# masa-ue/SVDD

Measured on AMD Instinct MI355X. Metric: decoded sequences/sec (whole node), L=200 M=10 128-step SVDD-MC, higher is better.
Workload: dtype f32; 1 GPU; DNA enhancer SVDD-MC, batch=256/GPU, L=200, M=10, 128 steps (BASELINE.json configs[1]); dilated-CNN backbone 3.3M params + ConvGRU value net; global_batch=256, rng=philox

## Files before the change

### include/svdd_hip.h

```cpp
#ifndef SVDD_HIP_H
#define SVDD_HIP_H

#include <stdint.h>

#ifdef __cplusplus
extern "C" {
#endif

#define SVDD_VOCAB 5
#define SVDD_MASK 4
#define SVDD_MAX_M 1024

enum {
  SVDD_OK = 0,
  SVDD_E_ARG = -1,
  SVDD_E_LAUNCH = -2,
  SVDD_E_NODEVICE = -3
};

enum {
  SVDD_LAYOUT_BLV = 0,
  SVDD_LAYOUT_BVL = 1
};

// ... 134 lines not shown
int svdd_conv_tower_windows_f32(const float* onehot, const float* tiles, const float* bias, const int32_t* win,
                                const float* parent_out, float* out, int n, int L, int M, int nlayers,
                                int residual_mask, const int32_t* live_idx, const int32_t* count, void* stream);

int svdd_candidate_windows_tight(const uint8_t* cand, const uint8_t* x, int B, int L, int M, int margin, int32_t* win,
                                 int32_t* flags, void* on_stream);

int svdd_candidate_parts(const uint8_t* cand, const uint8_t* x, int B, int L, int M, int reach, int gap, int32_t* parts,
                         int32_t* nparts, int32_t* flags, int32_t* key, void* on_stream);
int svdd_conv_tower_parts_f32(const float* onehot, const float* tiles, const float* bias, const int32_t* parts,
                              const float* parent_out, float* out, int n, int L, int M, int nlayers, int residual_mask,
                              int reach, const int32_t* live_idx, const int32_t* count, void* on_stream);

int svdd_backbone_cnn_f32(const uint8_t* x, const float* table0, const float* tiles, const float* vec,
                          const float* w2, float* out, int n, int L, int nlayers, const int* dilations,
                          const int32_t* count, const int32_t* row_idx, int out_scatter, void* stream);
int svdd_backbone_cnn_save_f32(const uint8_t* x, const float* table0, const float* tiles, const float* vec, const float* w2,
                               float* out, int n, int L, int nlayers, const int* dilations, float* xhat, float* rstd,
                               unsigned long long* mask, void* stream);
int svdd_backbone_cnn_grad_f32(const float* dlogits, const float* tiles_bwd, const float* gamma, const float* w2,
                               const float* table0, const float* xhat, const float* rstd, const unsigned long long* mask,
                               float* dx, int n, int L, int nlayers, const int* dilations, void* stream);
int svdd_backbone_incr_f32(const uint8_t* x, const float* table0, const float* tiles, const float* vec, const float* w2,
                           float* out, int n, int L, int nlayers, const int* dilations, int lead, float* planes,
                           uint8_t* x_prev, int32_t* items, unsigned long long* stat, int first, int max_item, void* on_stream);
int svdd_backbone_incr2_f32(const uint8_t* x, const float* table0, const float* tiles, const float* vec, const float* w2,
                            float* out, int n, int L, int nlayers, const int* dilations, int lead, float* planes,
                            uint8_t* x_prev, int32_t* items, unsigned long long* stat, int first, int max_item,
                            int32_t* order, int32_t* order_count, void* on_stream);
int svdd_backbone_incr3_f32(const uint8_t* x, const float* table0, const float* tiles, const float* vec, const float* w2,
                            float* out, int n, int L, int nlayers, const int* dilations, int lead, float* planes,
                            uint8_t* x_prev, int32_t* items, unsigned long long* stat, int first, int max_item,
                            int32_t* order, int32_t* order_count, int depth, void* on_stream);
int svdd_backbone_incr_set_residency(int wg_per_cu);
int svdd_backbone_set_workspace(void* ws, long long bytes);
int svdd_backbone_split_status(int* err);

enum { SVDD_PREC_F32 = 0, SVDD_PREC_F16X3 = 1, SVDD_PREC_BF16X3 = 2, SVDD_PREC_F16 = 3, SVDD_PREC_BF16 = 4 };

int svdd_backbone_cnn_lp(const uint8_t* x, const float* table0, const void* tiles, const float* vec,
                         const float* lscale, const float* w2, float* out, int n, int L, int nlayers,
                         const int* dilations, int prec, const int32_t* count, const int32_t* row_idx, int out_scatter,
                         void* stream);

int svdd_conv_tower_lp(const uint8_t* tok, const void* tiles, const float* bias, const float* inv, void* out,
                       int n, int L, int nlayers, int residual_mask, const int32_t* count, int prec, void* stream);
int svdd_conv_tower_windows_lp(const uint8_t* cand, const void* tiles, const float* bias, const float* inv,
                               const int32_t* win, const void* parent_out, void* out, int n, int L, int M,
                               int nlayers, int residual_mask, const int32_t* live_idx, const int32_t* count,
                               int prec, void* stream);

int svdd_gru_bidir_lp(const float* x, const void* x16, const void* wpack, const float* bpack, const float* inv,
                      float* out, int n, int L, const int32_t* count, int prec, void* stream);

int svdd_value_tail_lp(const float* h_fwd, const float* h_bwd, const void* w1pack, const float* b1,
                       const float* w_eff, const float* b_eff, float inv, float* out, int n, int L, int n_tasks,
                       const int32_t* count, int prec, void* stream);

enum { SVDD_OPT_FORCE_EXACT = 0,
       SVDD_OPT_MSPLIT = 1 ,
       SVDD_OPT_SELECT_ONE_ROW = 2 ,
       SVDD_OPT_BACKBONE_LP_VERSION = 3 ,
       SVDD_OPT_TRUNK_GEMM_VERSION = 4 ,
       SVDD_OPT_CAND_ROW_STRIDE = 5 ,
       SVDD_OPT_TRUNK_PLANES_F32 = 6 ,
       SVDD_OPT_SELECT_BATCHES = 8 ,
// ... 60 lines not shown
```

### svdd_amd/_lib.py

```python
import ctypes
import os
import subprocess

_HERE = os.path.dirname(os.path.abspath(__file__))
CSRC = os.path.join(_HERE, "csrc")
SO_PATH = os.environ.get("SVDD_HIP_LIB") or os.path.join(CSRC, "libsvdd_hip.so")
ABI_VERSION = 17

OK, E_ARG, E_LAUNCH, E_NODEVICE = 0, -1, -2, -3
LAYOUT_BLV, LAYOUT_BVL = 0, 1
RNG_REPLAY, RNG_PHILOX = 0, 1
SELECT_ARGMAX, SELECT_MULTINOMIAL = 0, 1
TARGET_MEAN, TARGET_LOGMEANEXP = 0, 1
EVOLVE_GLOBAL, EVOLVE_ROW = 0, 1
ATTR_GRADIENT, ATTR_TIMES_INPUT = 0, 1
PRECISIONS = {"f32": 0, "f16x3": 1, "bf16x3": 2, "f16": 3, "bf16": 4}
MAX_M = 1024

OPT_FORCE_EXACT, OPT_MSPLIT, OPT_SELECT_ONE_ROW, OPT_BACKBONE_LP_VERSION, OPT_TRUNK_GEMM_VERSION = 0, 1, 2, 3, 4
OPT_CAND_ROW_STRIDE, OPT_TRUNK_PLANES_F32, OPT_BACKBONE_SPLIT, OPT_SELECT_BATCHES = 5, 6, 7, 8


class SvddRng(ctypes.Structure):
    _fields_ = [("kind", ctypes.c_int32), ("step", ctypes.c_uint32), ("uniforms", ctypes.c_void_p),
# ... 69 lines not shown
    "svdd_bb_layer_fwd_f32": (vp, vp, vp, vp, vp, vp, f32, vp, vp, vp, i64, i32, i32, STREAM),
    "svdd_bb_layer_bwd_f32": (vp, vp, vp, vp, f32, vp, vp, vp, vp, i64, i32, i32, STREAM),
    "svdd_mt19937_uniform_f32": (vp, vp, i64, STREAM),
    "svdd_backbone_set_workspace": (vp, i64),
    "svdd_backbone_split_status": (pi32,),
    "svdd_backbone_cnn_save_f32": (vp, vp, vp, vp, vp, vp, i32, i32, i32, pi32, vp, vp, vp, STREAM),
    "svdd_backbone_cnn_grad_f32": (vp, vp, vp, vp, vp, vp, vp, vp, vp, i32, i32, i32, pi32, STREAM),
    "svdd_dps_probs": (vp, vp, i32, i32, vp, STREAM),
    "svdd_dps_probs_bwd": (vp, vp, vp, i32, i32, vp, vp, STREAM),
    "svdd_dps_guided_q": (vp, vp, vp, vp, f32, f32, f32, i32, i32, vp, STREAM),
    "svdd_reward_stem_f32": (vp, vp, vp, vp, i32, i32, i32, STREAM),
    "svdd_reward_stem_bwd_f32": (vp, vp, vp, i32, i32, i32, STREAM),
    "svdd_conv1d_cl_gated_f32": (vp, vp, vp, i32, i32, i32, i32, i32, i32, vp, vp, STREAM),
    "svdd_reward_tail_grad_f32": (vp, vp, vp, vp, vp, vp, vp, f32, i32, i32, vp, vp, STREAM),
    "svdd_sum_gate_f32": (vp, vp, vp, vp, i64, STREAM),
    "svdd_gru_bidir_train2_f32": (vp, vp, vp, vp, vp, vp, i32, i32, STREAM),
    "svdd_gru_bidir_bwd2_f32": (vp, vp, vp, vp, vp, vp, vp, i32, i32, STREAM),
    "svdd_classifier_propose": (vp, i32, vp, vp, f32, f32, f32, i32, i32, RNG, vp, vp, vp, STREAM),
    "svdd_elbo_mask": (vp, i32, i32, i32, f64, RNG, vp, vp, vp, vp, vp, vp, STREAM),
    "svdd_elbo_nll": (vp, i32, vp, vp, vp, i32, i32, i32, vp, vp, vp, vp, STREAM),
    "svdd_refine_remask": (vp, vp, vp, vp, vp, f32, i32, i32, RNG, vp, vp, vp, vp, vp, vp, vp),
    "svdd_value_target": (vp, vp, i32, i32, i32, i32, f32, vp, vp, vp, vp),
    "svdd_ism_mutants": (vp, vp, vp, i32, i32, i32, vp, vp, vp, vp),
    "svdd_ism_fold": (vp, vp, vp, vp, vp, vp, i32, i32, i32, i32, i32, vp, vp, vp, vp, vp),
    "svdd_evolve_apply": (vp, vp, vp, i32, i32, i32, vp, vp, vp, vp, vp, vp, vp, vp, vp, vp, vp, vp),
    "svdd_attr_path": (vp, vp, i32, vp, i32, i32, i32, i32, i32, i32, vp, vp, vp),
    "svdd_attr_fold": (vp, f32, vp, vp, vp, i32, i32, i32, i32, i32, i32, i32, vp, vp, vp, vp),
    "svdd_candidate_windows_tight": (vp, vp, i32, i32, i32, i32, vp, vp, vp),
    "svdd_kmer_counts": (vp, i32, i32, i32, vp, vp, vp),
    "svdd_pack_tokens": (vp, i32, i32, vp, vp, vp),
    "svdd_hamming_nn": (vp, vp, i32, i32, i32, i32, i32, i32, vp, vp, vp),
    "svdd_candidate_parts": (vp, vp, i32, i32, i32, i32, i32, vp, vp, vp, vp, vp),
    "svdd_conv_tower_parts_f32": (vp, vp, vp, vp, vp, vp, i32, i32, i32, i32, i32, i32, vp, vp, vp),
}
EXPORTS = tuple(SIGNATURES)


def build(force=False):
    import glob
    srcs = sorted(glob.glob(os.path.join(CSRC, "*.hip")) + glob.glob(os.path.join(CSRC, "*.h")) + [os.path.join(CSRC, "Makefile")])
    srcs.append(os.path.join(os.path.dirname(_HERE), "include", "svdd_hip.h"))
    if os.environ.get("SVDD_HIP_LIB"):
        return SO_PATH
    stale = not os.path.exists(SO_PATH) or os.path.getmtime(SO_PATH) < max(os.path.getmtime(f) for f in srcs)
    if force or stale:
        subprocess.check_call(["make", "-C", CSRC, "-B", "-j", str(min(8, os.cpu_count() or 1))])
    return SO_PATH


_lib = None


def lib():
    global _lib
    if _lib is not None:
        return _lib
    import torch
    if not os.path.exists(SO_PATH):
        raise SvddError(f"{SO_PATH} is missing: build it with `python -c 'import __graft_entry__ as g; g.build()'` "
                        "or `make -C svdd_amd/csrc`. There is no CPU fallback for the SVDD hot path.")
    L = ctypes.CDLL(SO_PATH)
    for name in EXPORTS:
        if not hasattr(L, name):
            raise SvddError(f"libsvdd_hip.so does not export {name}")
    if L.svdd_abi_version() != ABI_VERSION:
        raise SvddError(f"libsvdd_hip.so ABI {L.svdd_abi_version()} != binding ABI {ABI_VERSION}; rebuild")
# ... 102 lines not shown
```

### svdd_amd/csrc/svdd_nets.hip

```cpp
#include "svdd_host.h"

namespace {

typedef float f32x4 __attribute__((ext_vector_type(4)));

__device__ __forceinline__ float wave_sum(float v) {
#pragma unroll
  for (int off = 32; off > 0; off >>= 1) v += __shfl_xor(v, off, 64);
  return v;
}


constexpr int H = 64;
constexpr int HPAD = H + 4;

__device__ __forceinline__ float sigmoid_fast(float a) {
  return __builtin_amdgcn_rcpf(1.0f + __builtin_amdgcn_exp2f(-1.44269504088896f * a));
}
__device__ __forceinline__ float tanh_fast(float a) {
  return 1.0f - 2.0f * __builtin_amdgcn_rcpf(1.0f + __builtin_amdgcn_exp2f(2.88539008177793f * a));
}

template <bool BOTH>
__global__ __launch_bounds__(BOTH ? 512 : 256) void gru_bidir_kernel(const float* __restrict__ x, const float* __restrict__ wpack,
// ... 1994 lines not shown
    int run = 0;
    for (int c = 0; c < 4; ++c) { base[c] = run; run += wtot[0][c] + wtot[1][c] + wtot[2][c] + wtot[3][c]; }
    order_count[blockIdx.x] = run;
  }
  __syncthreads();
  for (int r0 = 0; r0 < n; r0 += 256) {
    const int r = r0 + tid;
    int item[SLOTS], pos[4];
    for (int c = 0; c < 4; ++c) cnt[c] = 0;
    for (int s = 0; s < SLOTS; ++s) {
      item[s] = r < n ? it[r * SLOTS + s] : 0;
      for (int c = 0; c < 4; ++c) cnt[c] += (item[s] >> 8) == 4 - c;
    }
    for (int c = 0; c < 4; ++c) {
      int v = cnt[c];
#pragma unroll
      for (int off = 1; off < 64; off <<= 1) { const int u = __shfl_up(v, off, 64); if (lane >= off) v += u; }
      pos[c] = v - cnt[c];
      if (lane == 63) wtot[w][c] = v;
    }
    __syncthreads();
    for (int c = 0; c < 4; ++c) {
      int at = base[c] + pos[c];
      for (int q = 0; q < w; ++q) at += wtot[q][c];
      for (int s = 0; s < SLOTS; ++s)
        if ((item[s] >> 8) == 4 - c) ord[at++] = r << 16 | item[s];
    }
    __syncthreads();
    if (tid < 4) base[tid] += wtot[0][tid] + wtot[1][tid] + wtot[2][tid] + wtot[3][tid];
    __syncthreads();
  }
}

template <int NC, bool ORD = false, int DIL = 1>
__global__ __launch_bounds__(256, NC == 4 ? 2 : NC == 1 ? 4 : 3) void backbone_seg_kernel(BackboneSegArgs a) {
  static_assert(DIL == 1 || DIL == 4, "one halo tile per side holds taps of dilation <= 4");
  constexpr int NS = NC + 2, ROWS = 16 * NS;
  extern __shared__ __attribute__((aligned(16))) float smem[];
  float* img = smem;
  float* psum = img + ROWS * BB_AP;
  float* rstat = psum + 4 * ROWS;
  int* toks = reinterpret_cast<int*>(rstat + ROWS);

  int item, seq;
  if (ORD) {
    if ((int)blockIdx.x >= a.order_count[a.layer - 1]) return;
    const unsigned ent = (unsigned)__builtin_amdgcn_readfirstlane(a.order[(size_t)(a.layer - 1) * a.order_stride + blockIdx.x]);
    item = (int)(ent & 0xFFFFu);
    seq = (int)(ent >> 16);
  } else {
    item = __builtin_amdgcn_readfirstlane(a.items[(size_t)(a.layer - 1) * a.n * SEG_SLOTS + blockIdx.x]);
    seq = blockIdx.x / SEG_SLOTS;
  }
  const int nown = min(item >> 8, NC);
  if (nown == 0) return;
  const int t0 = item & 255;
  const int tid = threadIdx.x, lane = tid & 63;
  const int cg = __builtin_amdgcn_readfirstlane(tid >> 6);
  const int j = lane & 15, g = lane >> 4;
  const int col0 = 32 * cg + j;
  const int L = a.L;
  const int r0 = 16 * (t0 - 1);
  const size_t pl_stride = (size_t)a.n * TW_ROWS * BB_C;
  float* pl0 = a.planes + (size_t)seq * TW_ROWS * BB_C;
  const int cl = a.layer - 1;
#define SEG_LIVE(S) ((S) <= nown + 1)
// ... 176 lines not shown
        SG_MM(0, UC)                                                                                         \
      } else {                                                                                               \
        SG_MM(0, ua)                                                                                         \
        SG_ALOAD(0, ua, dbytes2)                                                                             \
        SG_MM(1, ub)                                                                                         \
        SG_ALOAD(1, ub, dbytes2)                                                                             \
      }                                                                                                      \
      ++it; }
  float4 ua[2], ub[2];
  SG_ALOAD(0, ua, SG_DBYTES(0))
  if constexpr (NC > 1) SG_ALOAD(1, ub, SG_DBYTES(0))
  for (int it = 0; it < 36;) {
    SG_ENTRY(bA, bB, ua, ub)
    SG_ENTRY(bB, bA, ub, ua)
  }
#undef SG_ENTRY
#undef SG_MM
#undef SG_ALOAD
#undef SG_DBYTES

  float* dst = pl0 + (size_t)cl * pl_stride;
#pragma unroll
  for (int c = 0; c < NC; ++c) {
    if (c >= nown) continue;
#pragma unroll
    for (int ct = 0; ct < 2; ++ct)
#pragma unroll
      for (int e = 0; e < 4; ++e) {
        const int row = r0 + 16 * (c + 1) + 4 * g + e;
        if (row < L) dst[row * BB_C + col0 + 16 * ct] = fmaxf(cacc[c][ct][e], 0.0f) + f[c + 1][ct][e];
      }
  }
#undef SEG_LIVE
}

struct BackboneGradArgs {
  const float* dlogits;
  const float* tiles;
  const float* gamma;
  const float* w2;
  const float* table0;
  float* dx;
  int n, L, nl;
  int dil[BB_MAXL];
};

__global__ __launch_bounds__(512, 2) void backbone_grad_kernel(BackboneGradArgs a, BackboneSave sv) {
  extern __shared__ __attribute__((aligned(16))) float smem[];
  float* img = smem + BB_AP;
  float* Bs = smem + (TW_ROWS + 2) * BB_AP;
  float* psum = Bs + 9 * 5 * BB_C;
  float* rstat = psum + 8 * TW_ROWS;
  int* sdil = reinterpret_cast<int*>(rstat + 2 * TW_ROWS);
  int* sched = sdil + BB_MAXL + 1;

  const int tid = threadIdx.x, lane = tid & 63;
  const int w = __builtin_amdgcn_readfirstlane(tid >> 6);
  const int cg = w & 3, rh = w >> 2;
  const int j = lane & 15, g = lane >> 4;
  const int col0 = 32 * cg + j;
  const int L = a.L, nl = a.nl;
  const int tile_rows = L;
  const int64_t row0 = (int64_t)blockIdx.x * L;
  const int it_end = (nl + 1) * 36;
  constexpr int NR = 7;

// ... 1001 lines not shown
  if (first) {
    if (hipMemcpyAsync(x_prev, x, (size_t)n * L, hipMemcpyDeviceToDevice, (hipStream_t)stream) != hipSuccess) return SVDD_E_LAUNCH;
    return svdd_launch_timed(span.all(), backbone_kernel<true, false, 1>, dim3((unsigned)n), dim3(512), lds, stream, a, BackboneSave{});
  }
  const int slots = max_item == 1 ? TW_RT : SEG_SLOTS;
  if (svdd_launch_timed(span.first(), max_item == 1 ? backbone_worklist_kernel<TW_RT> : backbone_worklist_kernel<SEG_SLOTS>,
                        dim3((unsigned)((n + 3) / 4)), dim3(256), 0, stream, x, x_prev, n, L, depth, max_item, items, stat,
                        backbone_reach(dilations, depth, lead)) != SVDD_OK)
    return SVDD_E_LAUNCH;
  if (svdd_launch(max_item == 1 ? backbone_order_kernel<TW_RT> : backbone_order_kernel<SEG_SLOTS>, dim3((unsigned)depth), dim3(256), 0, stream,
                  items, n, order, order_count) != SVDD_OK)
    return SVDD_E_LAUNCH;
  BackboneSegArgs sa{x, table0, tiles, vec, planes, items, n, L, 0, order, order_count, n * slots};
  const int rows = 16 * (max_item + 2);
  size_t slds = sizeof(float) * ((size_t)rows * BB_AP + 5 * (size_t)rows + rows + 8);
  if (g_incr_residency > 0) {
    const size_t pad = (CU_LDS_BYTES / (size_t)(g_incr_residency + 1) / 1024 + 1) * 1024;
    if (pad > slds) slds = pad;
  }
  const dim3 sgrid((unsigned)(n * slots));
  void (*seg1)(BackboneSegArgs) = max_item == 4 ? backbone_seg_kernel<4, true> : max_item == 2 ? backbone_seg_kernel<2, true>
                                                                                                 : backbone_seg_kernel<1, true>;
  void (*seg4)(BackboneSegArgs) = max_item == 4 ? backbone_seg_kernel<4, true, 4> : max_item == 2 ? backbone_seg_kernel<2, true, 4>
                                                                                                    : backbone_seg_kernel<1, true, 4>;
  svdd_raise_lds_limit(seg1, slds);
  if (depth > lead) svdd_raise_lds_limit(seg4, slds);
  for (int k = 1; k <= depth; ++k) {
    sa.layer = k;
    if (svdd_launch(k <= lead ? seg1 : seg4, sgrid, dim3(256), slds, stream, sa) != SVDD_OK) return SVDD_E_LAUNCH;
  }
  return svdd_launch_timed(span.last(), backbone_kernel<true, false, 2>, dim3((unsigned)n), dim3(512), lds, stream, a, BackboneSave{});
}

typedef decltype(&value_tail_kernel<1>) ValueTailKernel;

extern "C" int svdd_value_tail_f32(const float* h_fwd, const float* h_bwd, const float* w1pack, const float* b1,
                                   const float* w_eff, const float* b_eff, float* out, int n, int L, int n_tasks,
                                   const int32_t* count, void* stream) {
  if (!h_fwd || !h_bwd || !w1pack || !b1 || !w_eff || !b_eff || !out || n <= 0 || L <= 0 || n_tasks < 1 || n_tasks > 4)
    return SVDD_E_ARG;
  ValueTailKernel kern;
  switch (n_tasks) {
    case 1: kern = value_tail_kernel<1>; break;
    case 2: kern = value_tail_kernel<2>; break;
    case 3: kern = value_tail_kernel<3>; break;
    default: kern = value_tail_kernel<4>; break;
  }
  SvddSpan span(SVDD_SLOT_VALUE_TAIL);
  return svdd_launch_timed(span.all(), kern, dim3((unsigned)((n + 3) / 4)), dim3(256), 0, stream, h_fwd, h_bwd, w1pack, b1, w_eff, b_eff, out,
                           n, L, count);
}

extern "C" int svdd_candidate_windows(const uint8_t* cand, const uint8_t* x, int B, int L, int M, int margin, int32_t* win,
                                      int32_t* flags, void* stream) {
  if (!cand || !x || !win || B <= 0 || L <= 0 || M <= 0 || margin < 0) return SVDD_E_ARG;
  const int n = B * M;
  return svdd_launch(candidate_windows_kernel<false>, dim3((unsigned)((n + 3) / 4)), dim3(256), 0, stream, cand, x, n, L, M, margin, win, flags);
}

extern "C" int svdd_candidate_windows_tight(const uint8_t* cand, const uint8_t* x, int B, int L, int M, int margin, int32_t* win,
                                            int32_t* flags, void* on_stream) {
  if (!cand || !x || !win || B <= 0 || L <= 0 || M <= 0 || margin < 0 || margin > (1 << 20) ||
      (long long)B * M > 0x7fffffffLL)
    return SVDD_E_ARG;
  const int n = B * M;
  return svdd_launch(candidate_windows_kernel<true>, dim3((unsigned)((n + 3) / 4)), dim3(256), 0, on_stream, cand, x, n, L, M, margin, win, flags);
// ... 36 lines not shown
```

### svdd_amd/diffusion.py

```python
import contextlib
import functools
import math
import os
import warnings
import weakref
from dataclasses import dataclass
from typing import Optional

import numpy as np
import torch
import torch.nn.functional as F
from torch import nn

from . import noise_schedule, ops
from .backbone import CNNModel


@dataclass
class Loss:
    loss: torch.Tensor
    nlls: torch.Tensor
    token_mask: torch.Tensor


# ... 99 lines not shown
            self.backbone = CNNModel(config.model, alphabet_size=self.vocab_size, num_cls=3)
        elif config.backbone == "dit":
            from .dit import DIT
            self.backbone = DIT(config.model, vocab_size=self.vocab_size)
        else:
            raise ValueError(f"Unknown backbone: {config.backbone}")
        if self.parameterization != "subs":
            raise ValueError("only the `subs` parameterization is on the reference's decode path "
                             "(configs_gosai/config_gosai.yaml:13)")
        self.T = config.T
        self.subs_masking = config.subs_masking
        self.noise = noise_schedule.get_noise(config)
        self.time_conditioning = config.time_conditioning
        self.neg_infinity = -1000000.0
        self.sampling_eps = config.training.sampling_eps
        self.rng_mode = "replay"
        self.value_batching = "batched"
        self.select_mode = "argmax"
        self.philox_seed = 0
        self.row_offset = 0
        self._shard = None
        self.fuse_nets = True
        self.precision = "f32"
        self.skip_unchanged = True
        self.late_steps_from = "auto"
        self.dedup_prior = True
        self.dps_fused = True
        self.dps_one_launch = True
        self._dps_hard_onehot, self._dps_raw_logits, self._dps_logp = False, None, None
        self.dps_single_forward = False
        self.logits_cache = "auto"
        self.incremental_backbone = "auto"
        self.incremental_depth = os.environ.get("SVDD_INCR_DEPTH") or "auto"
        self.skip_stats = None
        self.skip_generic = False
        self.trace = None
        self.state_trace = None
        self._sched_cache = {}
        self._fused = WeightCache()
        self._scope_depth, self._scope_id = 0, 0
        self.fuse_trunk_f32 = True
        self.replay_rng = "device"
        self._replay_stream = None
        self._replay_checked = None
        self._classifier_fused_last = None
        self.elbo_trace = None
        self._from_state = False
        self.cdq_draws = 10
        self._step_base = 0

    @property
    def device(self):
        return next(self.parameters()).device

    def _require_gpu(self):
        if self.device.type != "cuda":
            raise ops.SvddError("the SVDD sampler runs on the GPU only (move the model with .cuda()); "
                                "there is no CPU fallback for the hot path")

    def _schedule(self, num_steps, eps, t_start=1.0):
        key = (num_steps, eps, float(t_start))
        if key not in self._sched_cache:
            tab, timesteps, dt = noise_schedule.move_chance_table(self.noise, num_steps, eps, float(t_start))
            self._sched_cache[key] = (tab.numpy().copy(), timesteps, dt)
        return self._sched_cache[key]

# ... 1137 lines not shown
        mode, rng = self._select_args(step)
        x_next, _, _, _ = ops.select_compact(sc, ws.slot, ws.parent_score, cand, mode=mode, rng=rng, sel_score=ws.sel_score,
                                             changed=ws.changed, idx=ws.idx)
        ws.parent_score, ws.sel_score = ws.sel_score, ws.parent_score
        if ws.parent_out is not None and ws.seq is not None:
            ops.advance_rows(ws.seq, ws.slot, ws.idx, ws.parent_out, ws.M)
        if self.skip_stats is not None:
            ws.n_live += ws.count
            ws.n_changed += ws.changed.sum()
        return x_next

    def _dense_scores(self, sc, ws, B, M):
        live = ws.slot >= 0
        return torch.where(live, sc[ws.slot.clamp(min=0).long()], ws.parent_score.repeat_interleave(M)).view(B, M)

    def _finish_stats(self, ws, B, M, S, kind):
        if self.skip_stats is not None:
            self.skip_stats.update(kind=kind, steps=S, candidates=B * M * S, live_candidates=int(ws.n_live),
                                   row_steps=B * S, changed_row_steps=int(ws.n_changed),
                                   tower_window_rows=None if ws.n_win_rows is None else int(round(float(ws.n_win_rows))),
                                   tower_tile_layers=None if ws.n_tile_layers is None else int(ws.n_tile_layers))

    def _use_logits_cache(self, L):
        return self.logits_cache == "on" or (self.logits_cache == "auto" and 208 // L >= 2)

    def _incremental_stem(self, B, L):
        if self.incremental_backbone not in ("auto", "on", "off"):
            raise ValueError(f"incremental_backbone = {self.incremental_backbone!r}: expected 'auto', 'on' or 'off'")
        if self.incremental_backbone == "off" or _capturing():
            return None, None
        fb = self._fused_backbone_or_none(L)
        if fb is None or not fb.incremental_ok(B, L, any_batch=self.incremental_backbone == "on"):
            return None, None
        return fb, fb.incremental_stem(B, L, self._incremental_depth(fb))

    def _incremental_depth(self, fb):
        from .fused import INCR_DEPTH_AUTO, leading_dilation1, following_dilation4
        lead = leading_dilation1(fb.ol_dil)
        most = lead + following_dilation4(fb.ol_dil)
        if self.incremental_depth == "auto":
            return min(max(INCR_DEPTH_AUTO, lead), most)
        try:
            depth = int(self.incremental_depth)
        except (TypeError, ValueError):
            depth = -1
        if not lead <= depth <= most:
            raise ValueError(f"incremental_depth = {self.incremental_depth!r}: expected 'auto' or {lead} .. {most}")
        return depth

    def _controlled_sample_skipping(self, fn, x, cand, onehot, sched, B, L, S, M):
        from .fused import candidate_windows
        ws = self._SkipWorkspace(B, M, self.device)
        if self.skip_stats is not None:
            ws.n_win_rows = torch.zeros(1, dtype=torch.float64, device=self.device)
            ws.n_tile_layers = torch.zeros(1, dtype=torch.int64, device=self.device)
        from .fused import FusedValueNet
        dedup = self._prior_dedup_ok(x) and isinstance(fn, FusedValueNet)
        ws.parent_score.copy_(fn.forward_tokens(x[:1].contiguous()).reshape(1).expand(B) if dedup
                              else fn.forward_tokens(x).reshape(B))
        ws.prior_rows_identical = dedup
        fb = self._fused_backbone_or_none(L) if self._use_logits_cache(L) else None
        share = hasattr(fn, "candidates_ok") and fn.candidates_ok(L, M)
        toks_c = None if share else torch.empty((B * M, L), dtype=torch.uint8, device=self.device)
        logits = None
        inc, stem = (None, None) if fb is not None else self._incremental_stem(B, L)
        if stem is not None:
            stem.stat.zero_()
# ... 293 lines not shown
```

### svdd_amd/fused.py

```python
import ctypes
import os
import math

import torch
import torch.nn.functional as F
from torch import nn

from . import _lib
from .backbone import CNNModel
from .value_nets import ConvGRUTrunk, ConvHead


def _cl(w):
    return w.detach().unsqueeze(2).contiguous(memory_format=torch.channels_last)


def pack_gru(gru):
    H = gru.hidden_size
    assert H == 64 and gru.input_size == 64 and gru.bidirectional and gru.num_layers == 1 and gru.bias
    packs, biases = [], []
    for sfx in ("", "_reverse"):
        w_ih = getattr(gru, "weight_ih_l0" + sfx).detach().float()
        w_hh = getattr(gru, "weight_hh_l0" + sfx).detach().float()
        b_ih = getattr(gru, "bias_ih_l0" + sfx).detach().float()
# ... 309 lines not shown
              row_idx, int(scatter))
    return out


INCR_MAX_ITEM = 2
INCR_ORDERED = True
INCR_RESIDENCY = 0
INCR_DEPTH_AUTO = 10
INCR_SLOTS = 13


def set_incr_residency(r):
    global INCR_RESIDENCY
    _lib.call("svdd_backbone_incr_set_residency", int(r))
    INCR_RESIDENCY = int(r)


def leading_dilation1(dil):
    n = 0
    while n < len(dil) and dil[n] == 1:
        n += 1
    return n


def following_dilation4(dil):
    lead = n = leading_dilation1(dil)
    while n < len(dil) and dil[n] == 4:
        n += 1
    return n - lead


class IncrementalStem:

    def __init__(self, n, L, lead, dev, deep=0):
        self.n, self.L, self.lead, self.deep = n, L, lead, deep
        depth = lead + deep
        self.planes = torch.empty((depth, n, 208, 128), dtype=torch.float32, device=dev)
        self.x_prev = torch.empty((n, L), dtype=torch.uint8, device=dev)
        self.items = torch.zeros((depth, n, INCR_SLOTS), dtype=torch.int32, device=dev)
        self.order = torch.zeros((depth, n * INCR_SLOTS), dtype=torch.int32, device=dev)
        self.order_count = torch.zeros(depth, dtype=torch.int32, device=dev)
        self.stat = torch.zeros(2, dtype=torch.int64, device=dev)
        self.valid = False
        self.forwards = 0


def backbone_cnn_incremental(tokens, pk, st, out=None, max_item=None):
    assert tokens.is_cuda and tokens.dtype == torch.uint8 and tokens.is_contiguous() and tuple(tokens.shape) == (st.n, st.L)
    n, L = tokens.shape
    if out is None:
        out = torch.empty((n, L, 5), dtype=torch.float32, device=tokens.device)
    dil = (ctypes.c_int * len(pk["dil"]))(*pk["dil"])
    first = not st.valid
    stream = ctypes.c_void_p(torch.cuda.current_stream().cuda_stream)
    if st.deep > 0:
        _lib.call("svdd_backbone_incr3_f32", tokens, pk["table0"], pk["tiles"], pk["vec"], pk["w2"], out, n, L, len(pk["dil"]), dil,
                  st.lead, st.planes, st.x_prev, st.items, st.stat, int(first), int(max_item or INCR_MAX_ITEM), st.order,
                  st.order_count, st.lead + st.deep, stream)
    elif INCR_ORDERED:
        _lib.call("svdd_backbone_incr2_f32", tokens, pk["table0"], pk["tiles"], pk["vec"], pk["w2"], out, n, L, len(pk["dil"]), dil,
                  st.lead, st.planes, st.x_prev, st.items, st.stat, int(first), int(max_item or INCR_MAX_ITEM), st.order,
                  st.order_count, stream)
    else:
        _lib.call("svdd_backbone_incr_f32", tokens, pk["table0"], pk["tiles"], pk["vec"], pk["w2"], out, n, L, len(pk["dil"]), dil,
                  st.lead, st.planes, st.x_prev, st.items, st.stat, int(first), int(max_item or INCR_MAX_ITEM), stream)
    st.valid = True
    st.forwards += 0 if first else 1
    return out


LP_DTYPES = {"f16x3": (torch.float16, 2), "bf16x3": (torch.bfloat16, 2), "f16": (torch.float16, 1), "bf16": (torch.bfloat16, 1)}


def _pow2_floor(v):
    return 2.0 ** math.floor(math.log2(v))


def _split16(w, dtype, parts):
    hi = w.to(dtype)
    if parts == 1:
        return hi.unsqueeze(-1)
    lo = (w - hi.float()).to(dtype)
    return torch.stack([hi, lo], dim=-1)


def pack_backbone_lp(cnn, precision):
    dtype, parts = LP_DTYPES[precision]
    pk = pack_backbone(cnn)
# ... 557 lines not shown
        self.min_tiles_one_launch = 0
        self.precision = "f32"
        self._cnn = (cnn,)
        self._lp = {}
        self._grad_pack = None
        self._incr = {}
        if self.one_launch:
            pk = pack_backbone(cnn)
            self.ol_dil = pk.pop("dil")
            for k, v in pk.items():
                self.register_buffer("ol_" + k, v, persistent=False)

    def ol_pack(self):
        return dict(table0=self.ol_table0, tiles=self.ol_tiles, vec=self.ol_vec, w2=self.ol_w2, dil=self.ol_dil)

    def grad_ok(self, L):
        return self.one_launch and self.use_one_launch and 104 < L <= 208

    def grad_pack(self):
        if self._grad_pack is None:
            self._grad_pack = {k: v.to(self.ol_tiles.device) for k, v in pack_backbone_grad(self._cnn[0]).items()}
        return self._grad_pack

    def forward_with_grad(self, x_onehot, tokens):
        return BackboneOneLaunchFunction.apply(x_onehot, tokens.contiguous(), self.ol_pack(), self.grad_pack())

    def kernel_ok(self, L):
        return self.one_launch and self.use_one_launch and L <= 208 and self.min_tiles_one_launch == 0

    def incremental_ok(self, n, L, any_batch=False):
        return (self.kernel_ok(L) and self.precision == "f32" and 104 < L <= 208 and leading_dilation1(self.ol_dil) >= 2 and
                (any_batch or (n > BB_SPLIT_MAX_SEQ and not 0 < n % 256 <= BB_SPLIT_MAX_SEQ)))

    def incremental_stem(self, n, L, depth=None):
        lead = leading_dilation1(self.ol_dil)
        deep = 0 if depth is None else int(depth) - lead
        if not 0 <= deep <= following_dilation4(self.ol_dil):
            raise ValueError(f"incremental depth {depth}: expected {lead} .. {lead + following_dilation4(self.ol_dil)}")
        key = (n, L, deep, self.ol_tiles.device)
        st = self._incr.get(key)
        if st is None:
            self._incr.clear()
            st = self._incr[key] = IncrementalStem(n, L, lead, self.ol_tiles.device, deep)
        st.valid = False
        return st

    def forward_incremental(self, tok, st, out=None):
        return backbone_cnn_incremental(tok, self.ol_pack(), st, out)

    def _lp_pack(self):
        pk = self._lp.get(self.precision)
        if pk is None:
            pk = self._lp[self.precision] = pack_backbone_lp(self._cnn[0], self.precision)
        return pk

    def forward_rows(self, tok, count=None, out=None, row_idx=None, scatter=False):
        if self.precision != "f32":
            return backbone_cnn_lp(tok, self._lp_pack(), count, out, row_idx, scatter)
        return backbone_cnn(tok, self.ol_pack(), count, out, row_idx, scatter)

    def forward(self, seq, sigma=None):
        B, L = seq.shape
        if self.precision != "f32" and self.one_launch and L <= 208 and seq.is_cuda:
            tok = seq if seq.dtype == torch.uint8 else seq.to(torch.uint8)
            return backbone_cnn_lp(tok.contiguous(), self._lp_pack())
        if (self.one_launch and self.use_one_launch and L <= 208 and seq.is_cuda and
                (B + 208 // L - 1) // (208 // L) >= self.min_tiles_one_launch):
            tok = seq if seq.dtype == torch.uint8 else seq.to(torch.uint8)
            return backbone_cnn(tok.contiguous(), self.ol_pack())
        onehot = self.eye[seq.long()]
        f = onehot.view(B, 1, L, onehot.shape[2]).permute(0, 3, 1, 2)
        n = len(self.ws)
        f, hn = epilogue_ln(F.conv2d(f, self.first_w, None, padding=(0, 4)), self.first_b, None,
                            self.tb[0], self.norms[0].weight, self.norms[0].bias)
        hip_conv = self.use_hip_conv and self.H == 128 and L in (200, 50) and B * L >= 192 * 200
        for i, (w, b) in enumerate(zip(self.ws, self.bs)):
            d = self.dil[i]
# ... 23 lines not shown
```

Measured before the change: 803.1 sequences/s.

## Add tight row-window incremental backbone path with double-buffered previous tokens

Adds a new incremental backbone entry point, enabled by default through a 'tight' items mode. For the leading dilation-1 layers, recompute windows now start at the changed rows instead of 16-row-aligned tiles, and a dedicated segment kernel handles these windows. A rewritten list kernel finds changed positions with 8-byte word compares and builds the items and order lists. The previous-token buffer is double-buffered by parity instead of being copied each step. The aim is to recompute fewer rows per denoising step and cut per-step overhead, at the cost of a more complex list build and an extra kernel variant that runs only when max_item is 2.

```diff
diff --git a/include/svdd_hip.h b/include/svdd_hip.h
--- a/include/svdd_hip.h
+++ b/include/svdd_hip.h
@@ -190,6 +190,10 @@
                             float* out, int n, int L, int nlayers, const int* dilations, int lead, float* planes,
                             uint8_t* x_prev, int32_t* items, unsigned long long* stat, int first, int max_item,
                             int32_t* order, int32_t* order_count, int depth, void* on_stream);
+int svdd_backbone_incr4_f32(const uint8_t* x, const float* table0, const float* tiles, const float* vec, const float* w2,
+                            float* out, int n, int L, int nlayers, const int* dilations, int lead, float* planes,
+                            uint8_t* x_prev, int32_t* items, unsigned long long* stat, int first, int max_item,
+                            int32_t* order, int32_t* order_count, int depth, uint8_t* x_prev2, int parity, void* on_stream);
 int svdd_backbone_incr_set_residency(int wg_per_cu);
 int svdd_backbone_set_workspace(void* ws, long long bytes);
 int svdd_backbone_split_status(int* err);
diff --git a/svdd_amd/_lib.py b/svdd_amd/_lib.py
--- a/svdd_amd/_lib.py
+++ b/svdd_amd/_lib.py
@@ -125,6 +125,7 @@
     "svdd_hamming_nn": (vp, vp, i32, i32, i32, i32, i32, i32, vp, vp, vp),
     "svdd_candidate_parts": (vp, vp, i32, i32, i32, i32, i32, vp, vp, vp, vp, vp),
     "svdd_conv_tower_parts_f32": (vp, vp, vp, vp, vp, vp, i32, i32, i32, i32, i32, i32, vp, vp, vp),
+    "svdd_backbone_incr4_f32": (vp, vp, vp, vp, vp, vp, i32, i32, i32, pi32, i32, vp, vp, vp, vp, i32, i32, vp, vp, i32, vp, i32, vp),
 }
 EXPORTS = tuple(SIGNATURES)
 
diff --git a/svdd_amd/csrc/svdd_nets.hip b/svdd_amd/csrc/svdd_nets.hip
--- a/svdd_amd/csrc/svdd_nets.hip
+++ b/svdd_amd/csrc/svdd_nets.hip
@@ -2050,6 +2050,165 @@
   }
 }
 
+__global__ __launch_bounds__(256) void backbone_list_kernel(const uint8_t* __restrict__ x, const uint8_t* __restrict__ x_cur,
+                                                            uint8_t* __restrict__ x_next, int n, int L, int max_item,
+                                                            int* __restrict__ items, int* __restrict__ order,
+                                                            int* __restrict__ order_count, unsigned long long* __restrict__ stat,
+                                                            BackboneReach rc) {
+  typedef unsigned long long u64;
+  __shared__ u64 chs[256][4];
+  __shared__ int its[256][SEG_SLOTS];
+  __shared__ int wtot[4][4];
+  __shared__ int base[4];
+  const int tid = threadIdx.x, lane = tid & 63, wave = tid >> 6;
+  const int reach = rc.r[blockIdx.x];
+  const bool tight = (int)blockIdx.x < rc.lead1, keep = blockIdx.x == 0;
+  int* itk = items + (size_t)blockIdx.x * n * SEG_SLOTS;
+  int* ord = order + (size_t)blockIdx.x * n * SEG_SLOTS;
+  const bool words = L % 8 == 0 && ((reinterpret_cast<uintptr_t>(x) | reinterpret_cast<uintptr_t>(x_cur) |
+                                     reinterpret_cast<uintptr_t>(x_next)) & 7) == 0;
+  unsigned char* chb = reinterpret_cast<unsigned char*>(chs);
+  const int half = lane >> 5, w8 = lane & 31;
+  int tiles = 0, item[SEG_SLOTS], cnt4[4] = {0, 0, 0, 0};
+  for (int r0 = 0; r0 < n; r0 += 256) {
+    if (words) {
+      u64 a[32], c[32];
+#pragma unroll
+      for (int i = 0; i < 32; ++i) {
+        const int rr = r0 + 64 * wave + 2 * i + half;
+        const bool in = rr < n && 8 * w8 < L;
+        const size_t at = in ? (size_t)rr * L + 8 * w8 : 0;
+        a[i] = *reinterpret_cast<const u64*>(x + at);
+        c[i] = *reinterpret_cast<const u64*>(x_cur + at);
+        if (!in) c[i] = a[i];
+      }
+#pragma unroll
+      for (int i = 0; i < 32; ++i) {
+        const int rl = 64 * wave + 2 * i + half;
+        if (keep && r0 + rl < n && 8 * w8 < L) *reinterpret_cast<u64*>(x_next + (size_t)(r0 + rl) * L + 8 * w8) = a[i];
+        const u64 d = a[i] ^ c[i];
+        const unsigned dl = (unsigned)d, dh = (unsigned)(d >> 32);
+        const unsigned zl = (((dl & 0x7F7F7F7Fu) + 0x7F7F7F7Fu) | dl) & 0x80808080u, zh = (((dh & 0x7F7F7F7Fu) + 0x7F7F7F7Fu) | dh) & 0x80808080u;
+        const unsigned m = ((zl >> 7) * 0x10204080u) >> 28 | (((zh >> 7) * 0x10204080u) >> 28) << 4;
+        chb[rl * 32 + w8] = (unsigned char)m;
+      }
+    } else {
+      for (int i = 0; i < 32; ++i) {
+        const int rl = 64 * wave + 2 * i + half, rr = r0 + rl;
+        unsigned m = 0;
+        if (rr < n)
+          for (int e = 0; e < 8 && 8 * w8 + e < L; ++e) {
+            const size_t at = (size_t)rr * L + 8 * w8 + e;
+            const uint8_t a = x[at];
+            if (keep) x_next[at] = a;
+            m |= (unsigned)(a != x_cur[at]) << e;
+          }
+        chb[rl * 32 + w8] = (unsigned char)m;
+      }
+    }
+    __syncthreads();
+    const int r = r0 + tid;
+    const u64 ch[4] = {chs[tid][0], chs[tid][1], chs[tid][2], chs[tid][3]};
+    int* it = its[tid];
+    int cnt = 0, nt = 0;
+    if (tight) {
+      int cend = -1, io = 0, il = 0;
+#pragma unroll
+      for (int q = 0; q < 4; ++q)
+        for (u64 b = ch[q]; b; b &= b - 1) {
+          const int p = 64 * q + __builtin_ctzll(b);
+          const int lo = max(0, p - reach), hi = min(L - 1, p + reach);
+          int o = lo > cend ? lo : cend + 1;
+          for (; o <= hi; o += 16) {
+            ++nt;
+            if (il > 0 && il < max_item && o == io + 16 * il) { ++il; continue; }
+            if (il > 0) { if (cnt < SEG_SLOTS) it[cnt] = io | il << 8; ++cnt; }
+            io = o; il = 1;
+          }
+          cend = o - 1;
+        }
+      if (il > 0) { if (cnt < SEG_SLOTS) it[cnt] = io | il << 8; ++cnt; }
+    }
+    if (!tight || cnt > SEG_SLOTS) {
+      int m = 0;
+#pragma unroll
+      for (int q = 0; q < 4; ++q)
+        for (u64 b = ch[q]; b; b &= b - 1) {
+          const int p = 64 * q + __builtin_ctzll(b);
+          const int tlo = max(0, p - reach) >> 4, thi = min(L - 1, p + reach) >> 4;
+          m |= ((2 << thi) - 1) & ~((1 << tlo) - 1);
+        }
+      cnt = 0; nt = __popc(m);
+      for (int t = 0; t < TW_RT;) {
+        if (!(m >> t & 1)) { ++t; continue; }
+        int len = 1;
+        while (len < max_item && t + len < TW_RT && (m >> (t + len) & 1)) ++len;
+        it[cnt++] = (tight ? 16 * t : t) | len << 8;
+        t += len;
+      }
+    }
+    for (; cnt < SEG_SLOTS; ++cnt) it[cnt] = 0;
+    tiles += nt;
+#pragma unroll
+    for (int s = 0; s < SEG_SLOTS; ++s) {
+      item[s] = its[tid][s];
+      if (r < n) itk[(size_t)r * SEG_SLOTS + s] = item[s];
+#pragma unroll
+      for (int c = 0; c < 4; ++c) cnt4[c] += (item[s] >> 8) == 4 - c;
+    }
+    __syncthreads();
+  }
+  if (stat) {
+#pragma unroll
+    for (int off = 32; off > 0; off >>= 1) tiles += __shfl_xor(tiles, off, 64);
+    if (lane == 0 && tiles) atomicAdd(stat + (tight ? 0 : 1), (unsigned long long)tiles);
+  }
+#pragma unroll
+  for (int c = 0; c < 4; ++c) {
+    int v = cnt4[c];
+#pragma unroll
+    for (int off = 32; off > 0; off >>= 1) v += __shfl_xor(v, off, 64);
+    if (lane == 0) wtot[wave][c] = v;
+  }
+  __syncthreads();
+  if (tid == 0) {
+    int run = 0;
+    for (int c = 0; c < 4; ++c) { base[c] = run; run += wtot[0][c] + wtot[1][c] + wtot[2][c] + wtot[3][c]; }
+    order_count[blockIdx.x] = run;
+  }
+  __syncthreads();
+  for (int r0 = 0; r0 < n; r0 += 256) {
+    const int r = r0 + tid;
+    int pos[4], cl[4] = {0, 0, 0, 0};
+#pragma unroll
+    for (int s = 0; s < SEG_SLOTS; ++s) {
+      if (n > 256) item[s] = r < n ? itk[(size_t)r * SEG_SLOTS + s] : 0;
+#pragma unroll
+      for (int c = 0; c < 4; ++c) cl[c] += (item[s] >> 8) == 4 - c;
+    }
+#pragma unroll
+    for (int c = 0; c < 4; ++c) {
+      int v = cl[c];
+#pragma unroll
+      for (int off = 1; off < 64; off <<= 1) { const int u = __shfl_up(v, off, 64); if (lane >= off) v += u; }
+      pos[c] = v - cl[c];
+      if (lane == 63) wtot[wave][c] = v;
+    }
+    __syncthreads();
+#pragma unroll
+    for (int c = 0; c < 4; ++c) {
+      int at = base[c] + pos[c];
+      for (int q = 0; q < wave; ++q) at += wtot[q][c];
+#pragma unroll
+      for (int s = 0; s < SEG_SLOTS; ++s)
+        if ((item[s] >> 8) == 4 - c) ord[at++] = r << 16 | item[s];
+    }
+    __syncthreads();
+    if (tid < 4) base[tid] += wtot[0][tid] + wtot[1][tid] + wtot[2][tid] + wtot[3][tid];
+    __syncthreads();
+  }
+}
+
 template <int NC, bool ORD = false, int DIL = 1>
 __global__ __launch_bounds__(256, NC == 4 ? 2 : NC == 1 ? 4 : 3) void backbone_seg_kernel(BackboneSegArgs a) {
   static_assert(DIL == 1 || DIL == 4, "one halo tile per side holds taps of dilation <= 4");
@@ -2292,6 +2451,221 @@
       }
   }
 #undef SEG_LIVE
+}
+
+__global__ __launch_bounds__(256, 5) void backbone_seg_tight_kernel(BackboneSegArgs a) {
+  constexpr int NC = 2, NS = NC + 1, PK = NC, ROWS = 16 * NC + 8;
+  extern __shared__ __attribute__((aligned(16))) float smem[];
+  float* img = smem;
+  float* psum = img + ROWS * BB_AP;
+  float* rstat = psum + 4 * ROWS;
+  int* toks = reinterpret_cast<int*>(rstat + ROWS);
+
+  if ((int)blockIdx.x >= a.order_count[a.layer - 1]) return;
+  const unsigned ent = (unsigned)__builtin_amdgcn_readfirstlane(a.order[(size_t)(a.layer - 1) * a.order_stride + blockIdx.x]);
+  const int item = (int)(ent & 0xFFFFu), seq = (int)(ent >> 16);
+  const int nown = min(item >> 8, NC);
+  if (nown == 0) return;
+  const int tid = threadIdx.x, lane = tid & 63;
+  const int cg = __builtin_amdgcn_readfirstlane(tid >> 6);
+  const int j = lane & 15, g = lane >> 4;
+  const int col0 = 32 * cg + j;
+  const int L = a.L;
+  const int r0 = (item & 255) - 4;
+  const int nrows = 16 * nown + 8;
+  const bool halo = g < 2;
+  const int hrow = g == 1 ? 16 * nown + 4 : 0;
+  const size_t pl_stride = (size_t)a.n * TW_ROWS * BB_C;
+  float* pl0 = a.planes + (size_t)seq * TW_ROWS * BB_C;
+  const int cl = a.layer - 1;
+#define SGT_LIVE(S) ((S) < nown || (S) == PK)
+#define SGT_MINE(S) ((S) < PK || halo)
+#define SGT_IROW(S) ((S) < PK ? 4 + 16 * (S) + 4 * g : hrow)
+
+  f32x4 f[NS][2], acc[NS][2];
+  if (a.layer == 1) {
+    for (int e = tid; e < nrows + 8; e += 256) {
+      const int p = r0 - 4 + e;
+      toks[e] = (p >= 0 && p < L) ? (int)a.x[(size_t)seq * L + p] : -1;
+    }
+    __syncthreads();
+    {
+      const int c = tid & (BB_C - 1);
+      const float b0 = a.vec[c];
+#pragma unroll 4
+      for (int ri = tid >> 7; ri < nrows; ri += 2) {
+        int tk[9];
+        float tv[9];
+#pragma unroll
+        for (int t = 0; t < 9; ++t) {
+          tk[t] = toks[ri + t];
+          tv[t] = a.table0[(unsigned)((t * 5 + max(tk[t], 0)) * BB_C + c)];
+        }
+        float v = b0;
+#pragma unroll
+        for (int t = 0; t < 9; ++t) v = tk[t] >= 0 ? v + tv[t] : v;
+        const int row = r0 + ri;
+        img[ri * BB_AP + c] = (row >= 0 && row < L) ? fmaxf(v, 0.0f) : 0.0f;
+      }
+    }
+    __syncthreads();
+#pragma unroll
+    for (int s = 0; s < NS; ++s) {
+      if (!SGT_LIVE(s)) continue;
+#pragma unroll
+      for (int ct = 0; ct < 2; ++ct)
+#pragma unroll
+        for (int e = 0; e < 4; ++e) f[s][ct][e] = SGT_MINE(s) ? img[(SGT_IROW(s) + e) * BB_AP + col0 + 16 * ct] : 0.0f;
+    }
+  } else {
+    const float* src = pl0 + (size_t)(a.layer - 2) * pl_stride;
+#pragma unroll
+    for (int s = 0; s < NS; ++s) {
+      if (!SGT_LIVE(s)) continue;
+#pragma unroll
+      for (int ct = 0; ct < 2; ++ct)
+#pragma unroll
+        for (int e = 0; e < 4; ++e) {
+          const int row = r0 + SGT_IROW(s) + e;
+          f[s][ct][e] = (SGT_MINE(s) && row >= 0 && row < L) ? src[row * BB_C + col0 + 16 * ct] : 0.0f;
+        }
+    }
+  }
+
+  const float* vl = a.vec + (size_t)(cl + 1) * 4 * BB_C;
+  {
+    const float tb0 = vl[BB_C + col0], tb1 = vl[BB_C + col0 + 16];
+#pragma unroll
+    for (int s = 0; s < NS; ++s) {
+      if (!SGT_LIVE(s)) continue;
+#pragma unroll
+      for (int e = 0; e < 4; ++e) {
+        const float sm = group16_sum((f[s][0][e] + tb0) + (f[s][1][e] + tb1));
+        if (j == 0 && SGT_MINE(s)) psum[cg * ROWS + SGT_IROW(s) + e] = sm;
+      }
+    }
+    __syncthreads();
+    if (tid < nrows)
+      rstat[tid] = ((psum[tid] + psum[ROWS + tid]) + (psum[2 * ROWS + tid] + psum[3 * ROWS + tid])) * (1.0f / BB_C);
+    __syncthreads();
+#pragma unroll
+    for (int s = 0; s < NS; ++s) {
+      if (!SGT_LIVE(s)) continue;
+      const float4 cur4 = *reinterpret_cast<const float4*>(rstat + SGT_IROW(s));
+      const float mean4[4] = {cur4.x, cur4.y, cur4.z, cur4.w};
+#pragma unroll
+      for (int e = 0; e < 4; ++e) {
+        const float mean = mean4[e];
+        const float d0 = f[s][0][e] + tb0 - mean, d1 = f[s][1][e] + tb1 - mean;
+        acc[s][0][e] = d0; acc[s][1][e] = d1;
+        const float sq = group16_sum(d0 * d0 + d1 * d1);
+        if (j == 0 && SGT_MINE(s)) psum[cg * ROWS + SGT_IROW(s) + e] = sq;
+      }
+    }
+    __syncthreads();
+    if (tid < nrows)
+      rstat[tid] = rsqrtf(((psum[tid] + psum[ROWS + tid]) + (psum[2 * ROWS + tid] + psum[3 * ROWS + tid])) * (1.0f / BB_C) + 1e-5f);
+    __syncthreads();
+    const float gm0 = vl[2 * BB_C + col0], gm1 = vl[2 * BB_C + col0 + 16];
+    const float bt0 = vl[3 * BB_C + col0], bt1 = vl[3 * BB_C + col0 + 16];
+#pragma unroll
+    for (int s = 0; s < NS; ++s) {
+      if (!SGT_LIVE(s)) continue;
+      const float4 cur4 = *reinterpret_cast<const float4*>(rstat + SGT_IROW(s));
+      const float rs4[4] = {cur4.x, cur4.y, cur4.z, cur4.w};
+#pragma unroll
+      for (int e = 0; e < 4; ++e) {
+        const int ri = SGT_IROW(s) + e, row = r0 + ri;
+        const float rs = rs4[e];
+        const bool in = row >= 0 && row < L;
+        if (SGT_MINE(s)) {
+          img[ri * BB_AP + col0] = in ? acc[s][0][e] * rs * gm0 + bt0 : 0.0f;
+          img[ri * BB_AP + col0 + 16] = in ? acc[s][1][e] * rs * gm1 + bt1 : 0.0f;
+        }
+      }
+    }
+  }
+
+  const float bl0 = vl[col0], bl1 = vl[col0 + 16];
+  f32x4 cacc[NC][2];
+#pragma unroll
+  for (int c = 0; c < NC; ++c) { cacc[c][0] = f32x4{bl0, bl0, bl0, bl0}; cacc[c][1] = f32x4{bl1, bl1, bl1, bl1}; }
+  typedef __attribute__((address_space(3))) f32x4 LdsF4;
+  const int img_lds = (int)(unsigned)(size_t)(const __attribute__((address_space(3))) float*)img;
+  const int arow0 = img_lds + (j * BB_AP + 8 * g) * 4;
+  const float* wsrc = a.tiles + (size_t)cl * 36 * BB_C * CH + col0 * CH + 8 * g;
+  const int live = (1 << nown) - 1;
+  float4 bA[4], bB[4];
+  bA[0] = *reinterpret_cast<const float4*>(wsrc);
+  bA[1] = *reinterpret_cast<const float4*>(wsrc + 4);
+  bA[2] = *reinterpret_cast<const float4*>(wsrc + 16 * CH);
+  bA[3] = *reinterpret_cast<const float4*>(wsrc + 16 * CH + 4);
+  bB[0] = bA[0]; bB[1] = bA[1]; bB[2] = bA[2]; bB[3] = bA[3];
+  __syncthreads();
+#define SGT_DBYTES(IT) (((IT) % 9) * (BB_AP * 4) + ((IT) / 9) * (CH * 4))
+#define SGT_ALOAD(C, V, DBYTES)                                                                              \
+      { const LdsF4* ap_ = reinterpret_cast<const LdsF4*>(arow0 + (DBYTES) + (C) * (16 * BB_AP * 4));         \
+        const f32x4 t0_ = ap_[0], t1_ = ap_[1];                                                              \
+        V[0] = make_float4(t0_[0], t0_[1], t0_[2], t0_[3]); V[1] = make_float4(t1_[0], t1_[1], t1_[2], t1_[3]); }
+#define SGT_MM(C, U)                                                                                         \
+      __builtin_amdgcn_sched_barrier(0);                                                                     \
+      __builtin_amdgcn_s_waitcnt(0xC07F | (2 << 8));       \
+      if (live & (1 << (C))) {                                                                               \
+        _Pragma("unroll") for (int q = 0; q < 2; ++q) {                                                      \
+          cacc[C][0] = __builtin_amdgcn_mfma_f32_16x16x4f32(U[q].x, bf0[4 * q], cacc[C][0], 0, 0, 0);        \
+          cacc[C][1] = __builtin_amdgcn_mfma_f32_16x16x4f32(U[q].x, bf1[4 * q], cacc[C][1], 0, 0, 0);        \
+          cacc[C][0] = __builtin_amdgcn_mfma_f32_16x16x4f32(U[q].y, bf0[4 * q + 1], cacc[C][0], 0, 0, 0);    \
+          cacc[C][1] = __builtin_amdgcn_mfma_f32_16x16x4f32(U[q].y, bf1[4 * q + 1], cacc[C][1], 0, 0, 0);    \
+          cacc[C][0] = __builtin_amdgcn_mfma_f32_16x16x4f32(U[q].z, bf0[4 * q + 2], cacc[C][0], 0, 0, 0);    \
+          cacc[C][1] = __builtin_amdgcn_mfma_f32_16x16x4f32(U[q].z, bf1[4 * q + 2], cacc[C][1], 0, 0, 0);    \
+          cacc[C][0] = __builtin_amdgcn_mfma_f32_16x16x4f32(U[q].w, bf0[4 * q + 3], cacc[C][0], 0, 0, 0);    \
+          cacc[C][1] = __builtin_amdgcn_mfma_f32_16x16x4f32(U[q].w, bf1[4 * q + 3], cacc[C][1], 0, 0, 0);    \
+        }                                                                                                    \
+      }                                                                                                      \
+      __builtin_amdgcn_sched_barrier(0);
+#define SGT_ENTRY(BC, BN)                                                                                    \
+    { const int nxt = it + 1 < 36 ? it + 1 : it;                                                             \
+      const float bf0[8] = {BC[0].x, BC[0].y, BC[0].z, BC[0].w, BC[1].x, BC[1].y, BC[1].z, BC[1].w};         \
+      const float bf1[8] = {BC[2].x, BC[2].y, BC[2].z, BC[2].w, BC[3].x, BC[3].y, BC[3].z, BC[3].w};         \
+      { const float* src = wsrc + (size_t)nxt * BB_C * CH;                                                   \
+        BN[0] = *reinterpret_cast<const float4*>(src);                                                       \
+        BN[1] = *reinterpret_cast<const float4*>(src + 4);                                                   \
+        BN[2] = *reinterpret_cast<const float4*>(src + 16 * CH);                                             \
+        BN[3] = *reinterpret_cast<const float4*>(src + 16 * CH + 4);                                         \
+      }                                                                                                      \
+      const int dbytes2 = SGT_DBYTES(nxt);                                                                   \
+      SGT_MM(0, ua)                                                                                          \
+      SGT_ALOAD(0, ua, dbytes2)                                                                              \
+      SGT_MM(1, ub)                                                                                          \
+      SGT_ALOAD(1, ub, dbytes2)                                                                              \
+      ++it; }
+  float4 ua[2], ub[2];
+  SGT_ALOAD(0, ua, SGT_DBYTES(0))
+  SGT_ALOAD(1, ub, SGT_DBYTES(0))
+  for (int it = 0; it < 36;) {
+    SGT_ENTRY(bA, bB)
+    SGT_ENTRY(bB, bA)
+  }
+#undef SGT_ENTRY
+#undef SGT_MM
+#undef SGT_ALOAD
+#undef SGT_DBYTES
+
+  float* dst = pl0 + (size_t)cl * pl_stride;
+#pragma unroll
+  for (int c = 0; c < NC; ++c) {
+    if (c >= nown) continue;
+#pragma unroll
+    for (int ct = 0; ct < 2; ++ct)
+#pragma unroll
+      for (int e = 0; e < 4; ++e) {
+        const int row = r0 + 4 + 16 * c + 4 * g + e;
+        if (row < L) dst[row * BB_C + col0 + 16 * ct] = fmaxf(cacc[c][ct][e], 0.0f) + f[c][ct][e];
+      }
+  }
+#undef SGT_LIVE
+#undef SGT_MINE
+#undef SGT_IROW
 }
 
 struct BackboneGradArgs {
@@ -3359,6 +3733,52 @@
   return svdd_launch_timed(span.last(), backbone_kernel<true, false, 2>, dim3((unsigned)n), dim3(512), lds, stream, a, BackboneSave{});
 }
 
+extern "C" int svdd_backbone_incr4_f32(const uint8_t* x, const float* table0, const float* tiles, const float* vec, const float* w2,
+                                       float* out, int n, int L, int nlayers, const int* dilations, int lead, float* planes,
+                                       uint8_t* x_prev, int32_t* items, unsigned long long* stat, int first, int max_item,
+                                       int32_t* order, int32_t* order_count, int depth, uint8_t* x_prev2, int parity,
+                                       void* on_stream) {
+  if (!x || !table0 || !tiles || !vec || !w2 || !out || !dilations || !planes || !x_prev || !items || !order || !order_count ||
+      !x_prev2 || x_prev2 == x_prev || n <= 0 || n > 65536 || L <= TW_ROWS / 2 || L > TW_ROWS || nlayers <= 0 || nlayers > BB_MAXL ||
+      lead < 2 || lead > nlayers || max_item != 2 || depth < lead || depth > nlayers || (parity != 0 && parity != 1))
+    return SVDD_E_ARG;
+  for (int i = 0; i < depth; ++i) if (dilations[i] != (i < lead ? 1 : 4)) return SVDD_E_ARG;
+  BackboneArgs a;
+  if (!backbone_args(a, x, table0, tiles, vec, w2, out, n, L, 1, nlayers, dilations)) return SVDD_E_ARG;
+  a.planes = planes; a.planes_P = depth;
+  hipStream_t stream = (hipStream_t)on_stream;
+  uint8_t* x_cur = parity ? x_prev2 : x_prev;
+  uint8_t* x_next = parity ? x_prev : x_prev2;
+  const SvddLds lds = svdd_lds_raised(backbone_lds_bytes(nlayers, 3));
+  SvddSpan span(SVDD_SLOT_BACKBONE);
+  if (first) {
+    if (hipMemcpyAsync(x_cur, x, (size_t)n * L, hipMemcpyDeviceToDevice, stream) != hipSuccess) return SVDD_E_LAUNCH;
+    return svdd_launch_timed(span.all(), backbone_kernel<true, false, 1>, dim3((unsigned)n), dim3(512), lds, stream, a, BackboneSave{});
+  }
+  if (svdd_launch_timed(span.first(), backbone_list_kernel, dim3((unsigned)depth), dim3(256), 0, stream, x, (const uint8_t*)x_cur, x_next, n,
+                        L, max_item, items, order, order_count, stat, backbone_reach(dilations, depth, lead)) != SVDD_OK)
+    return SVDD_E_LAUNCH;
+  BackboneSegArgs sa{x, table0, tiles, vec, planes, items, n, L, 0, order, order_count, n * SEG_SLOTS};
+  const int rows1 = 16 * max_item + 8, rows4 = 16 * (max_item + 2);
+  size_t slds1 = sizeof(float) * ((size_t)rows1 * BB_AP + 5 * (size_t)rows1 + rows1 + 8);
+  size_t slds4 = sizeof(float) * ((size_t)rows4 * BB_AP + 5 * (size_t)rows4 + rows4 + 8);
+  if (g_incr_residency > 0) {
+    const size_t pad = (CU_LDS_BYTES / (size_t)(g_incr_residency + 1) / 1024 + 1) * 1024;
+    if (pad > slds1) slds1 = pad;
+    if (pad > slds4) slds4 = pad;
+  }
+  const dim3 sgrid((unsigned)(n * SEG_SLOTS));
+  void (*seg1)(BackboneSegArgs) = backbone_seg_tight_kernel;
+  void (*seg4)(BackboneSegArgs) = backbone_seg_kernel<2, true, 4>;
+  svdd_raise_lds_limit(seg1, slds1);
+  if (depth > lead) svdd_raise_lds_limit(seg4, slds4);
+  for (int k = 1; k <= depth; ++k) {
+    sa.layer = k;
+    if (svdd_launch(k <= lead ? seg1 : seg4, sgrid, dim3(256), k <= lead ? slds1 : slds4, stream, sa) != SVDD_OK) return SVDD_E_LAUNCH;
+  }
+  return svdd_launch_timed(span.last(), backbone_kernel<true, false, 2>, dim3((unsigned)n), dim3(512), lds, stream, a, BackboneSave{});
+}
+
 typedef decltype(&value_tail_kernel<1>) ValueTailKernel;
 
 extern "C" int svdd_value_tail_f32(const float* h_fwd, const float* h_bwd, const float* w1pack, const float* b1,
diff --git a/svdd_amd/diffusion.py b/svdd_amd/diffusion.py
--- a/svdd_amd/diffusion.py
+++ b/svdd_amd/diffusion.py
@@ -155,6 +155,7 @@
         self.logits_cache = "auto"
         self.incremental_backbone = "auto"
         self.incremental_depth = os.environ.get("SVDD_INCR_DEPTH") or "auto"
+        self.incremental_items = os.environ.get("SVDD_INCR_ITEMS") or "tight"
         self.skip_stats = None
         self.skip_generic = False
         self.trace = None
@@ -1358,7 +1359,9 @@
         fb = self._fused_backbone_or_none(L)
         if fb is None or not fb.incremental_ok(B, L, any_batch=self.incremental_backbone == "on"):
             return None, None
-        return fb, fb.incremental_stem(B, L, self._incremental_depth(fb))
+        if self.incremental_items not in ("tight", "aligned"):
+            raise ValueError(f"incremental_items = {self.incremental_items!r}: expected 'tight' or 'aligned'")
+        return fb, fb.incremental_stem(B, L, self._incremental_depth(fb), tight=self.incremental_items == "tight")
 
     def _incremental_depth(self, fb):
         from .fused import INCR_DEPTH_AUTO, leading_dilation1, following_dilation4
diff --git a/svdd_amd/fused.py b/svdd_amd/fused.py
--- a/svdd_amd/fused.py
+++ b/svdd_amd/fused.py
@@ -365,11 +365,13 @@
 
 class IncrementalStem:
 
-    def __init__(self, n, L, lead, dev, deep=0):
-        self.n, self.L, self.lead, self.deep = n, L, lead, deep
+    def __init__(self, n, L, lead, dev, deep=0, tight=False):
+        self.n, self.L, self.lead, self.deep, self.tight = n, L, lead, deep, tight
         depth = lead + deep
         self.planes = torch.empty((depth, n, 208, 128), dtype=torch.float32, device=dev)
         self.x_prev = torch.empty((n, L), dtype=torch.uint8, device=dev)
+        self.x_prev2 = torch.empty((n, L), dtype=torch.uint8, device=dev)
+        self.parity = 0
         self.items = torch.zeros((depth, n, INCR_SLOTS), dtype=torch.int32, device=dev)
         self.order = torch.zeros((depth, n * INCR_SLOTS), dtype=torch.int32, device=dev)
         self.order_count = torch.zeros(depth, dtype=torch.int32, device=dev)
@@ -386,7 +388,12 @@
     dil = (ctypes.c_int * len(pk["dil"]))(*pk["dil"])
     first = not st.valid
     stream = ctypes.c_void_p(torch.cuda.current_stream().cuda_stream)
-    if st.deep > 0:
+    if st.tight and int(max_item or INCR_MAX_ITEM) == 2:
+        _lib.call("svdd_backbone_incr4_f32", tokens, pk["table0"], pk["tiles"], pk["vec"], pk["w2"], out, n, L, len(pk["dil"]), dil,
+                  st.lead, st.planes, st.x_prev, st.items, st.stat, int(first), 2, st.order, st.order_count, st.lead + st.deep,
+                  st.x_prev2, st.parity, stream)
+        st.parity ^= 0 if first else 1
+    elif st.deep > 0:
         _lib.call("svdd_backbone_incr3_f32", tokens, pk["table0"], pk["tiles"], pk["vec"], pk["w2"], out, n, L, len(pk["dil"]), dil,
                   st.lead, st.planes, st.x_prev, st.items, st.stat, int(first), int(max_item or INCR_MAX_ITEM), st.order,
                   st.order_count, st.lead + st.deep, stream)
@@ -1010,7 +1017,7 @@
         return (self.kernel_ok(L) and self.precision == "f32" and 104 < L <= 208 and leading_dilation1(self.ol_dil) >= 2 and
                 (any_batch or (n > BB_SPLIT_MAX_SEQ and not 0 < n % 256 <= BB_SPLIT_MAX_SEQ)))
 
-    def incremental_stem(self, n, L, depth=None):
+    def incremental_stem(self, n, L, depth=None, tight=False):
         lead = leading_dilation1(self.ol_dil)
         deep = 0 if depth is None else int(depth) - lead
         if not 0 <= deep <= following_dilation4(self.ol_dil):
@@ -1020,7 +1027,7 @@
         if st is None:
             self._incr.clear()
             st = self._incr[key] = IncrementalStem(n, L, lead, self.ol_tiles.device, deep)
-        st.valid = False
+        st.valid, st.tight = False, bool(tight)
         return st
 
     def forward_incremental(self, tok, st, out=None):
```

After: 811.5 sequences/s, median of 6. 1.01x the previous value.
